# WangYuTum/odometry

Measured on AMD Instinct MI355X. Metric: tracked frames/sec (1241x376, 4-level pyramid), higher is better.
Workload: dtype f32

## Files before the change

### include/odometry_hip.h

```cpp
#ifndef ODOMETRY_HIP_H
#define ODOMETRY_HIP_H

#include <stddef.h>
#include <stdint.h>

#ifdef __cplusplus
extern "C" {
#endif

typedef struct odo_ctx odo_ctx;
typedef struct odo_pyr odo_pyr;
typedef struct odo_lm odo_lm;
typedef struct odo_depth odo_depth;
typedef struct odo_tracker odo_tracker;
typedef struct odo_camera odo_camera;
typedef struct odo_map odo_map;
typedef struct odo_volume odo_volume;
typedef struct odo_rgbd_frontend odo_rgbd_frontend;

typedef struct {
  float f0, cx0, cy0;
} odo_intrinsics;

enum { ODO_PYR_IMAGE = 0, ODO_PYR_DEPTH = 1 };
// ... 69 lines not shown
int odo_lm_time_eval(odo_lm* lm, const odo_pyr* kf_img, const odo_pyr* kf_dep, const odo_pyr* cur_img, int level,
                     const float T_colmajor[16], int reps, float* mean_us, float* min_us, double* algorithmic_bytes,
                     int* n_points);
int odo_lm_time_eval_batch(int n, odo_lm* const* lms, const odo_pyr* const* kf_img, const odo_pyr* const* kf_dep,
                           const odo_pyr* const* cur_img, int level, const float T_colmajor[16], int reps, float* mean_us,
                           float* min_us, double* algorithmic_bytes, int* n_points_total);
int odo_lm_event_timing(odo_lm* lm, int on);
int odo_lm_event_stats(odo_lm* lm, double* total_us, long* launches, long* active_launches,
                       double* algorithmic_bytes);
int odo_lm_event_stats2(odo_lm* lm, double* coarse_us, long* coarse_launches);
int odo_lm_event_stats_ex(odo_lm* lm, double out[12]);
enum { ODO_SAMPLE_FLOOR = 0, ODO_SAMPLE_BILINEAR = 1 };
int odo_lm_set_sampling(odo_lm* lm, int sampling);
int odo_lm_set_mode(odo_lm* lm, int mode);
int odo_lm_points(const odo_lm* lm, int npts[ODO_MAX_LEVELS], int use_list[ODO_MAX_LEVELS]);
int odo_lm_launch_stats(const odo_lm* lm, int* n_active_launches, int* n_total_launches, double* algorithmic_bytes);
int odo_lm_persistent_stats(const odo_lm* lm, int* workgroups, int* fallbacks);
int odo_lm_persistent_backoff(const odo_lm* lm, int* strikes, int* retry_after, int* solves_until_retry);
int odo_lm_tdist_stats(odo_lm* lm, long* multi_launches, int* fallbacks);

int odo_debug_update_stamps(odo_lm* lm, const odo_pyr* kf_img, const odo_pyr* kf_dep, const odo_pyr* cur_img, int level,
                            const float T_colmajor[16], unsigned long long stamps[8]);
int odo_debug_solve(odo_ctx* ctx, const double acc[ODO_NACC], float lambda, float delta[6]);

int odo_depth_create(odo_ctx* ctx, float grad_th, float ssd_th, float photo_th, float min_depth, float max_depth,
                     float lambda, float huber_delta, float precision, int max_iters, int boundary,
                     const odo_intrinsics* K, float baseline, int max_residuals, int max_disparity, int any_size,
                     odo_depth** out);
int odo_depth_compute(odo_depth* d, const float* left, const float* right, int rows, int cols, uint8_t* val,
                      float* disp, float* dep);
// ... 208 lines not shown
```

### odometry_amd/_lib.py

```python
import ctypes as C
import os

_HERE = os.path.dirname(os.path.abspath(__file__))
LIB_PATH = os.environ.get("ODOMETRY_HIP_LIB") or os.path.join(_HERE, "lib", "libodometry_hip.so")

MAX_LEVELS = 8
NACC = 29
PYR_IMAGE, PYR_DEPTH = 0, 1


class Intrinsics(C.Structure):
    _fields_ = [("f0", C.c_float), ("cx0", C.c_float), ("cy0", C.c_float)]


class LmTraceRow(C.Structure):
    _fields_ = [("level", C.c_int), ("iter", C.c_int), ("n_res", C.c_int), ("accepted", C.c_int), ("stop", C.c_int),
                ("err", C.c_float), ("lambda_after", C.c_float), ("delta", C.c_float * 6)]


class TrackerParams(C.Structure):
    _fields_ = [("rows", C.c_int), ("cols", C.c_int), ("levels", C.c_int),
                ("lm_lambda", C.c_float), ("lm_precision", C.c_float), ("lm_max_iters", C.c_int * MAX_LEVELS),
                ("lm_robust", C.c_int), ("lm_huber_delta", C.c_float),
                ("grad_th", C.c_float), ("ssd_th", C.c_float), ("photo_th", C.c_float),
# ... 81 lines not shown
    "odo_lm_trace": (C.c_int, [_vp, C.POINTER(LmTraceRow), C.c_int, _ip]),
    "odo_lm_set_record": (C.c_int, [_vp, C.c_int]),
    "odo_lm_time_eval": (C.c_int, [_vp, _vp, _vp, _vp, C.c_int, _fp, C.c_int, _fp, _fp, _dp, _ip]),
    "odo_lm_time_eval_batch": (C.c_int, [C.c_int, C.POINTER(_vp), C.POINTER(_vp), C.POINTER(_vp), C.POINTER(_vp), C.c_int, _fp, C.c_int, _fp, _fp, _dp, _ip]),
    "odo_lm_event_timing": (C.c_int, [_vp, C.c_int]),
    "odo_lm_event_stats": (C.c_int, [_vp, _dp, C.POINTER(C.c_long), C.POINTER(C.c_long), _dp]),
    "odo_lm_event_stats2": (C.c_int, [_vp, _dp, C.POINTER(C.c_long)]),
    "odo_lm_event_stats_ex": (C.c_int, [_vp, _dp]),
    "odo_lm_solve_begin": (C.c_int, [_vp, _vp, _vp, _vp]),
    "odo_lm_set_idle_callback": (C.c_int, [_vp, _vp, _vp]),
    "odo_lm_candidate_begin": (C.c_int, [_vp, _vp, _vp, _vp, C.c_ulong]),
    "odo_lm_solve_batch": (C.c_int, [C.c_int, C.POINTER(_vp), C.POINTER(_vp), C.POINTER(_vp), C.POINTER(_vp), _fp, C.POINTER(C.c_int)]),
    "odo_lm_set_sampling": (C.c_int, [_vp, C.c_int]),
    "odo_lm_set_mode": (C.c_int, [_vp, C.c_int]),
    "odo_lm_points": (C.c_int, [_vp, _ip, _ip]),
    "odo_lm_launch_stats": (C.c_int, [_vp, _ip, _ip, _dp]),
    "odo_lm_persistent_stats": (C.c_int, [_vp, _ip, _ip]),
    "odo_lm_persistent_backoff": (C.c_int, [_vp, _ip, _ip, _ip]),
    "odo_lm_tdist_stats": (C.c_int, [_vp, C.POINTER(C.c_long), _ip]),
    "odo_debug_update_stamps": (C.c_int, [_vp, _vp, _vp, _vp, C.c_int, _fp, C.POINTER(C.c_ulonglong)]),
    "odo_debug_solve": (C.c_int, [_vp, _dp, C.c_float, _fp]),
    "odo_depth_create": (C.c_int, [_vp] + [C.c_float] * 8 + [C.c_int, C.c_int, C.POINTER(Intrinsics), C.c_float,
                                                          C.c_int, C.c_int, C.c_int, C.POINTER(_vp)]),
    "odo_depth_compute": (C.c_int, [_vp, _fp, _fp, C.c_int, C.c_int, _u8p, _fp, _fp]),
    "odo_depth_compute_dev": (C.c_int, [_vp, _vp, _vp, C.c_int, C.c_int, _vp, _vp, _vp]),
    "odo_depth_prepare_left_dev": (C.c_int, [_vp, _vp, _vp, C.c_int, C.c_int, C.c_ulonglong]),
    "odo_depth_prepare_left_dev_marked": (C.c_int, [_vp, _vp, _vp, C.c_int, C.c_int, C.c_ulonglong, C.c_ulong]),
    "odo_depth_compute_dev_stamped": (C.c_int, [_vp, _vp, _vp, C.c_int, C.c_int, _vp, _vp, _vp, C.c_ulonglong]),
    "odo_depth_compute_begin_dev": (C.c_int, [_vp, _vp, _vp, _vp, C.c_int, C.c_int, _vp, _vp, _vp, C.c_ulonglong, C.c_ulonglong, C.c_ulong]),
    "odo_depth_compute_end_dev": (C.c_int, [_vp, _vp, _vp, C.c_int, C.c_int, _vp, _vp, _vp, C.c_ulonglong, C.c_ulonglong]),
# ... 134 lines not shown
```

### odometry_amd/api.py

```python
import ctypes as C

import numpy as np

from . import _lib as L

_default_ctx = None


class Context:

    def __init__(self, device=0):
        lib = L.load()
        h = C.c_void_p()
        L.check(lib.odo_ctx_create(device, C.byref(h)), "odo_ctx_create")
        self.h = h
        self.lib = lib

    def synchronize(self):
        L.check(self.lib.odo_ctx_synchronize(self.h), "odo_ctx_synchronize")

    def timer_start(self):
        L.check(self.lib.odo_ctx_timer_start(self.h), "timer_start")

    def timer_stop(self):
# ... 193 lines not shown
        L.check(self.ctx.lib.odo_lm_time_eval(self.h, kImagePyr1.h, kDepthPyr1.h, kImagePyr2.h, level, _fp(Tc), reps,
                                              C.byref(mean), C.byref(mn), C.byref(b), C.byref(n)), "odo_lm_time_eval")
        return dict(mean_us=mean.value, min_us=mn.value, bytes=b.value, n_points=n.value)

    def set_sampling(self, bilinear):
        L.check(self.ctx.lib.odo_lm_set_sampling(self.h, 1 if bilinear else 0), "odo_lm_set_sampling")

    def set_mode(self, mode):
        L.check(self.ctx.lib.odo_lm_set_mode(self.h, mode), "odo_lm_set_mode")

    def points(self):
        n = (C.c_int * L.MAX_LEVELS)()
        u = (C.c_int * L.MAX_LEVELS)()
        L.check(self.ctx.lib.odo_lm_points(self.h, n, u), "odo_lm_points")
        return list(n)[:self.n_levels], list(u)[:self.n_levels]

    def launch_stats(self):
        a, t, b = C.c_int(0), C.c_int(0), C.c_double(0)
        L.check(self.ctx.lib.odo_lm_launch_stats(self.h, C.byref(a), C.byref(t), C.byref(b)), "odo_lm_launch_stats")
        return a.value, t.value, b.value

    def persistent_stats(self):
        k, f = C.c_int(0), C.c_int(0)
        L.check(self.ctx.lib.odo_lm_persistent_stats(self.h, C.byref(k), C.byref(f)), "odo_lm_persistent_stats")
        return k.value, f.value

    def tdist_stats(self):
        a, b = C.c_long(0), C.c_int(0)
        L.check(self.ctx.lib.odo_lm_tdist_stats(self.h, C.byref(a), C.byref(b)), "odo_lm_tdist_stats")
        return a.value, b.value
# ... 1055 lines not shown
```

### odometry_amd/csrc/kernels.hip.h

```cpp
#pragma once
#include <hip/hip_runtime.h>
#include "odo_math.h"

#ifndef ODO_PHASE_STAMPS
#define ODO_PHASE_STAMPS 0
#endif
#if ODO_PHASE_STAMPS
#define ODO_DBG(a) ((a).dbg)
#else
#define ODO_DBG(a) ((unsigned long long*)nullptr)
#endif

#ifndef ODO_KERNEL
#define ODO_KERNEL __global__
#define ODO_KERNEL_T __global__
#endif
#ifdef ODO_LM_CHAIN_TU
#define ODO_DEVICE_VAR static __device__
#else
#define ODO_DEVICE_VAR __device__
#endif

namespace odo {

// ... 493 lines not shown
  const int px = (ui - 1 >= 0) ? ui - 1 : 0, nx = (ui + 1 < cols) ? ui + 1 : cols - 1;
  const int py = (vi - 1 >= 0) ? vi - 1 : 0, ny = (vi + 1 < rows) ? vi + 1 : rows - 1;
  const unsigned row = (unsigned)vi * (unsigned)cols, ucols = (unsigned)cols;
  const float tc = ldg_f32(I2_uniform, (row + (unsigned)ui) * 4u), tl = ldg_f32(I2_uniform, (row + (unsigned)px) * 4u),
              tr = ldg_f32(I2_uniform, (row + (unsigned)nx) * 4u), tu = ldg_f32(I2_uniform, ((unsigned)py * ucols + (unsigned)ui) * 4u),
              td = ldg_f32(I2_uniform, ((unsigned)ny * ucols + (unsigned)ui) * 4u);
  const float gx = 0.5f * (tr - tl), gy = 0.5f * (td - tu);
  *r = tc - p.i1;
  J[0] = gx * p.fx_z;
  J[1] = gy * p.fx_z;
  J[2] = gx * p.jw02 + gy * p.jw12;
  J[3] = gx * p.jw03 + gy * p.jw13;
  J[4] = gx * p.jw04 + gy * p.jw14;
  J[5] = gx * p.jw05 + gy * p.jw15;
  return true;
}

ODO_KERNEL void __launch_bounds__(kLmBlock) lm_residual_list_kernel(PointList pl, int n, const float* __restrict__ I2, int rows,
                                                                     int cols, LevelK k, const LmState* __restrict__ st,
                                                                     int expect_level, int robust, float huber_delta,
                                                                     const float* __restrict__ scale_sqr_ptr,
                                                                     double* __restrict__ partials) {
  if (!(st->active != 0 && st->level == expect_level)) return;
  float T[16];
#pragma unroll
  for (int i = 0; i < 16; i++) T[i] = st->T[i];
  const float scale_sqr = (robust == 2) ? *scale_sqr_ptr : 1.0f;
  double acc[ODO_NACC];
#pragma unroll
  for (int q = 0; q < ODO_NACC; q++) acc[q] = 0.0;
// ... 248 lines not shown
template <int T, int S>
__device__ __forceinline__ double rows_accumulate(const float* __restrict__ rows, int rowA, int rowB, int s, double acc) {
  static_assert(S == kRowSub && (T / S) % 4 == 0, "the row layout is built for S sub-lanes");
  constexpr int W = RowBuf<T>::W;
  const float4* A = (const float4*)(rows + rowA * W + s * RowBuf<T>::kStride);
  const float4* B = (const float4*)(rows + rowB * W + s * RowBuf<T>::kStride);
#pragma unroll
  for (int i = 0; i < T / S / 4; i++) {
    const float4 a = A[i], b = B[i];
    acc = fma((double)a.x, (double)b.x, acc);
    acc = fma((double)a.y, (double)b.y, acc);
    acc = fma((double)a.z, (double)b.z, acc);
    acc = fma((double)a.w, (double)b.w, acc);
  }
  return acc;
}

__device__ __forceinline__ double wave_sum64(double v) {
  v += dpp_d<0xB1>(v);
  v += dpp_d<0x4E>(v);
  v += dpp_d<0x141>(v);
  v += dpp_d<0x140>(v);
  const double r0 = readlane_d(v, 0), r1 = readlane_d(v, 16), r2 = readlane_d(v, 32), r3 = readlane_d(v, 48);
  return (r0 + r1) + (r2 + r3);
}
__device__ __forceinline__ float tdist_term(float e2, float sigma_sqr) { return e2 * (1.0f + 200.0f) / (200.0f + e2 / sigma_sqr); }
__device__ __forceinline__ float tdist_next_sigma(double total, int n) { return sqrtf((float)(total / (double)n)); }
__device__ __forceinline__ bool tdist_converged(float nxt, float cur) { return !(fabsf(nxt - cur) >= 1e-3f); }
constexpr int kTdistMaxPasses = 1000;

// ... 625 lines not shown
ODO_KERNEL void __launch_bounds__(kLmBlock) lm_step_kernel(StepArgs a) {
  const StepLaunch q = {a.st_in, a.st_out, a.part_in, a.part_out, a.seq, a.first_of_solve, a.span};
  lm_step_body(a, q);
}
ODO_KERNEL void __launch_bounds__(kLmBlock) lm_step_kernel_batch(const StepArgs* __restrict__ table, int seq, int first_of_solve,
                                                                 unsigned long long* span) {
  const StepArgs& a = table[blockIdx.y];
  const StepLaunch q = {a.st2[seq & 1], a.st2[(seq + 1) & 1], a.part2[seq & 1], a.part2[(seq + 1) & 1], seq, first_of_solve, span};
  lm_step_body(a, q);
}

#ifndef ODO_COARSE_BLOCK
#define ODO_COARSE_BLOCK 512
#endif
constexpr int kCoarseBlock = ODO_COARSE_BLOCK;
constexpr int kCoarseLdsBytes = 2 * RowBuf<kLmBlock>::kBytes;
constexpr int kCoarseMaxPoints = 1024;

constexpr int kCoarseRounds = kCoarseMaxPoints / kCoarseBlock;
constexpr int kCoarseChunks = kCoarseRounds * (kCoarseBlock / kWave);
__device__ __forceinline__ float coarse_tdist_sigma(double (*part)[kCoarseChunks], int* cnt, const float e2[kCoarseRounds],
                                                    const bool valid[kCoarseRounds], int nr) {
  constexpr int kW = kCoarseBlock / kWave;
  const int lane = threadIdx.x & 63, wv = threadIdx.x >> 6;
  int my_cnt[kCoarseRounds];
#pragma unroll
  for (int rd = 0; rd < kCoarseRounds; rd++) my_cnt[rd] = __popcll(__ballot(rd < nr && valid[rd]));
  float sigma = 5.0f;
  int n_total = 0;
  for (int pass = 0; pass < kTdistMaxPasses; pass++) {
#pragma unroll
// ... 76 lines not shown
    __syncthreads();
  }
#if ODO_PHASE_STAMPS
  const unsigned long long w_p1 = (unsigned long long)wall_clock64();
#endif
  lm_fused_prologue(q.st_in, q.part_in, lv_sh, a.n_levels, a.lambda0, a.precision, s_sh, red_sh, acc_sh, (kFull ? a.trace : (LmTraceRow*)nullptr), a.cost_stat, true,
                    kArmed ? arm_pose_sh : (q.first_of_solve ? a.init : nullptr), a.stop_level, (!kArmed && a.chain_in_token) ? a.chain_pose : nullptr);
#if ODO_PHASE_STAMPS
  const unsigned long long w_p2 = (unsigned long long)wall_clock64();
#endif
  LmHot hot;
  lm_hot_load(hot, s_sh);
  if (ODO_DBG(a) && threadIdx.x == 0 && q.seq < 56) ODO_DBG(a)[16 + 2 * q.seq] = wall_clock64();
  unsigned long long c_eval = 0, c_red = 0, c_sm = 0, c_it = 0, c_last = ODO_DBG(a) ? __builtin_readcyclecounter() : 0;
  const unsigned long long c_begin = c_last, w_begin = ODO_DBG(a) ? (unsigned long long)wall_clock64() : 0;
  auto lap = [&](unsigned long long& sum) {
    if (ODO_DBG(a)) { const unsigned long long now = __builtin_readcyclecounter(); sum += now - c_last; c_last = now; }
  };
  static_assert(kCoarseBlock == 2 * kLmBlock, "two 256-point virtual blocks per round");
  constexpr int kS = 8;
  constexpr int kVbMax = (kCoarseMaxPoints + kLmBlock - 1) / kLmBlock;
  __shared__ double part_sh[kVbMax][32];
  __shared__ double sc_part[2][kCoarseChunks];
  __shared__ int sc_cnt[kCoarseChunks];
  const int tl = threadIdx.x & (kLmBlock - 1), half = threadIdx.x >> 8;
  float* rows_sh = (float*)red_sh + half * (kRowFloats * RowBuf<kLmBlock>::W);
  const int my_q = tl / kS, my_s = tl % kS;
  int rowA = 0, rowB = 0;
  if (my_q < ODO_NACC) rows_of_quantity(my_q, &rowA, &rowB);
  PointK cpt[kCoarseRounds];
  bool cpt_ok[kCoarseRounds] = {false, false};
  int cpt_level = -1;
  for (int guard = 0; guard < 4096; guard++) {
    const bool run = (s_sh.active != 0 && s_sh.status == 0 && s_sh.level >= min_level);
    if (!run) break;
    c_it++;
    const StepLevel& L = lv_sh[s_sh.level];
    const float* I2u = lm_uniform_ptr(L.I2);
    float T[16];
#pragma unroll
    for (int i = 0; i < 16; i++) T[i] = s_sh.T[i];
    const int nvb = L.nblk;
    if (s_sh.level != cpt_level) {
      cpt_level = s_sh.level;
#pragma unroll
      for (int rd = 0; rd < kCoarseRounds; rd++) {
        const int vb = 2 * rd + half, idx = vb * kLmBlock + tl;
        cpt_ok[rd] = vb < nvb && idx < L.n;
        if (cpt_ok[rd]) cpt[rd] = load_point(L.pl, idx);
      }
    }
    float td_r[kCoarseRounds] = {0.0f, 0.0f}, td_J[kCoarseRounds][6] = {{0.0f, 0.0f, 0.0f, 0.0f, 0.0f, 0.0f}, {0.0f, 0.0f, 0.0f, 0.0f, 0.0f, 0.0f}};
    bool td_valid[kCoarseRounds] = {false, false};
    float td_scale_sqr = 1.0f;
    if ((kFull && a.robust == 2)) {
      float e2[kCoarseRounds];
#pragma unroll
      for (int rd = 0; rd < kCoarseRounds; rd++) {
        if (cpt_ok[rd]) td_valid[rd] = point_residual_g<kFull>(cpt[rd], T, L.k, I2u, L.rows, L.cols, &td_r[rd], td_J[rd]);
        e2[rd] = td_r[rd] * td_r[rd];
      }
      const float sg = coarse_tdist_sigma(sc_part, sc_cnt, e2, td_valid, (nvb + 1) / 2);
      td_scale_sqr = sg * sg;
    }
#pragma unroll
    for (int vb0 = 0; vb0 < 2 * kCoarseRounds; vb0 += 2) {
      if (vb0 >= nvb) break;
      const int vb = vb0 + half;
      float r = 0.0f, w = 0.0f, J[6] = {0.0f, 0.0f, 0.0f, 0.0f, 0.0f, 0.0f};
      bool valid = false;
      if ((kFull && a.robust == 2)) {
        r = td_r[vb0 / 2]; valid = td_valid[vb0 / 2];
#pragma unroll
        for (int i = 0; i < 6; i++) J[i] = td_J[vb0 / 2][i];
        if (valid) w = robust_weight(r, 2, a.huber_delta, td_scale_sqr);
      } else if (cpt_ok[vb0 / 2]) {
        if (point_residual_g<kFull>(cpt[vb0 / 2], T, L.k, I2u, L.rows, L.cols, &r, J)) {
          w = robust_weight(r, kFull ? a.robust : (a.robust == 1 ? 1 : 0), a.huber_delta, 1.0f);
          valid = true;
        }
      }
      if (vb0 > 0) __syncthreads();
      rows_store_z(rows_sh, RowBuf<kLmBlock>::W, tl, J, w, r, valid);
      __syncthreads();
      if (vb0 == 0) lap(c_eval);
      double accq = 0.0;
      if (vb < nvb) {
        if (my_q < ODO_NACC) accq = rows_accumulate<kLmBlock, kS>(rows_sh, rowA, rowB, my_s, accq);
        accq = rows_butterfly8(accq);
      }
      if (nvb == 1) {
        if (half == 0 && my_q < ODO_NACC && my_s == 0) {
          double v = 0.0;
          v += accq;
          double acc = 0.0;
          acc += v;
#pragma unroll
          for (int g = 1; g < 8; g++) acc += 0.0;
          acc_sh[my_q] = acc;
        }
      } else if (vb < nvb && my_q < ODO_NACC && my_s == 0) {
        part_sh[vb][my_q] = accq;
      }
    }
    __syncthreads();
    if (nvb > 1) {
      const int fq = threadIdx.x & 31, fseg = threadIdx.x >> 5;
      double* fold_sh = red_sh;
      if (fseg < 8) {
        double v = 0.0;
        if (fq < ODO_NACC)
          for (int b = fseg; b < nvb; b += 8) v += part_sh[b][fq];
        fold_sh[fseg * 32 + fq] = v;
      }
      __syncthreads();
      if (threadIdx.x < ODO_NACC) {
        double acc = 0.0;
// ... 12 lines not shown
#endif
  if (threadIdx.x == 0) lm_hot_store(hot, s_sh);
  lm_fused_publish(s_sh, q.st_out, a.host_prog, q.seq, a.token, a.cost_stat, a.out, a.done_flag, a.final_state, chain_out_of(a));
#if ODO_PHASE_STAMPS
  if (ODO_DBG(a) && threadIdx.x == 0) {
    const unsigned long long now = (unsigned long long)wall_clock64();
    g_lm_diag[4] += w_begin - w_entry; g_lm_diag[5] += w_loop_end - w_begin; g_lm_diag[6] += now - w_loop_end;
    g_lm_diag[16] += w_p1 - w_entry; g_lm_diag[17] += w_p2 - w_p1; g_lm_diag[18] += w_begin - w_p2;
    if (g_lm_diag[1] && w_entry > g_lm_diag[1] && w_entry - g_lm_diag[1] < 100000ull) { g_lm_diag[7] += w_entry - g_lm_diag[1]; g_lm_diag[3] += w_entry - g_lm_diag[2]; g_lm_diag[14] += 1; }
    g_lm_diag[0] = now; g_lm_diag[8] += 1;
  }
#endif
  if (ODO_DBG(a) && threadIdx.x == 0) {
    if (q.seq < 56) ODO_DBG(a)[16 + 2 * q.seq + 1] = wall_clock64();
    ODO_DBG(a)[0] += c_eval; ODO_DBG(a)[1] += c_red; ODO_DBG(a)[2] += c_sm; ODO_DBG(a)[3] += c_it;
    ODO_DBG(a)[4] += __builtin_readcyclecounter() - c_begin; ODO_DBG(a)[5] += 1;
    ODO_DBG(a)[6] += (unsigned long long)wall_clock64() - w_begin;
#pragma unroll
    for (int i = 0; i < 4; i++) ODO_DBG(a)[8 + i] += sm_sh[i];
  }
  lm_span_end(q.span);
}

#ifdef ODO_LM_CHAIN_TU
static __global__ void __launch_bounds__(kCoarseBlock) lm_coarse_kernel(StepArgs a, int min_level) {
  const StepLaunch q = {a.st_in, a.st_out, a.part_in, a.part_out, a.seq, a.first_of_solve, a.span};
  lm_coarse_body<false>(a, q, min_level, lm_kernarg_words());
}
static __global__ void __launch_bounds__(kCoarseBlock) lm_coarse_armed_kernel(StepArgs a, int min_level) {
  const StepLaunch q = {a.st_in, a.st_out, a.part_in, a.part_out, a.seq, a.first_of_solve, a.span};
// ... 275 lines not shown
  __syncthreads();
  const bool local = local_sh != 0;
  constexpr int kS = 8;
  const int my_q = tl / kS, my_s = tl % kS;
  int rowA = 0, rowB = 0;
  if (my_q < ODO_NACC) rows_of_quantity(my_q, &rowA, &rowB);
  const int fq = t & 31, fseg = t >> 5;
  PointK pt;
  bool pt_ok = false;
  int pt_level = -1;
  unsigned long long c_eval = 0, c_xchg = 0, c_sm = 0, c_it = 0, c_last = ODO_DBG(a) ? __builtin_readcyclecounter() : 0;
#if ODO_PHASE_STAMPS
  unsigned long long c_first = 0, n_first = 0;
#endif
  const unsigned long long c_begin = c_last, w_begin = ODO_DBG(a) ? (unsigned long long)wall_clock64() : 0;
  auto lap = [&](unsigned long long& sum) {
    if (ODO_DBG(a)) { const unsigned long long now = __builtin_readcyclecounter(); sum += now - c_last; c_last = now; }
  };
  for (int ev = 0; ev < 4096; ev++) {
    const bool run = (s_sh.active != 0 && s_sh.status == 0 && !s_sh.finished && !bail_sh && s_sh.level >= lo_level);
    if (!run) break;
    c_it++;
    const StepLevel& L = lv_sh[s_sh.level];
    const float* I2u = lm_uniform_ptr(L.I2);
    const int nblk = L.nblk;
    const unsigned tag = tag_base + 1u + (unsigned)(ev % 255);
    unsigned long long* buf = xbuf + (size_t)(ev & 1) * kFineRowsMax * kFineGran;
    float T[16];
#pragma unroll
    for (int i = 0; i < 16; i++) T[i] = s_sh.T[i];
#if ODO_PHASE_STAMPS
    const bool first_of_level = (s_sh.level != pt_level);
#endif
    const bool resident = (nblk <= 2 * K) && (L.n <= nblk * kLmBlock);
    if (resident) {
      const int vb = w + half * K;
      if (s_sh.level != pt_level) {
// ... 102 lines not shown
  }
#if ODO_PHASE_STAMPS
  const unsigned long long w_loop_end = (unsigned long long)wall_clock64();
#endif
  if (t == 0) lm_hot_store(hot, s_sh);
  if (bail_sh && t == 0) { s_sh.status = -2; s_sh.active = 0; s_sh.finished = 1; }
  __syncthreads();
  if (publisher) {
    lm_fused_publish(s_sh, q.st_out, a.host_prog, q.seq, a.token, a.cost_stat, a.out, a.done_flag, a.final_state, chain_out_of(a));
#if ODO_PHASE_STAMPS
    const unsigned long long w_published = (unsigned long long)wall_clock64();
#endif
    if (ODO_DBG(a) && t == 0) { ODO_DBG(a)[128] += c_eval; ODO_DBG(a)[129] += c_xchg; ODO_DBG(a)[130] += c_sm; ODO_DBG(a)[131] += c_it; ODO_DBG(a)[132] += 1; ODO_DBG(a)[133] += local ? 1 : 0;
      ODO_DBG(a)[134] += __builtin_readcyclecounter() - c_begin; ODO_DBG(a)[135] += (unsigned long long)wall_clock64() - w_begin;
#pragma unroll
      for (int i = 0; i < 4; i++) ODO_DBG(a)[136 + i] += sm_sh[i]; }
    if (t == 0 && q.span) atomicMax(q.span + 1, (unsigned long long)wall_clock64());
#if ODO_PHASE_STAMPS
    if (ODO_DBG(a) && t == 0) {
      const unsigned long long now = w_published;
      g_lm_diag[2] = w_loop_end;
      g_lm_diag[19] += c_first; g_lm_diag[20] += n_first;
      g_lm_diag[9] += w_begin - w_entry; g_lm_diag[10] += w_loop_end - w_begin; g_lm_diag[11] += now - w_loop_end;
      if (g_lm_diag[0] && w_entry > g_lm_diag[0] && w_entry - g_lm_diag[0] < 100000ull) { g_lm_diag[12] += w_entry - g_lm_diag[0]; g_lm_diag[15] += 1; }
      g_lm_diag[1] = now; g_lm_diag[13] += 1;
    }
#endif
  }
}
ODO_DEVICE_VAR unsigned g_lm_fine_dispatch[2];
__device__ __forceinline__ bool lm_fine_mid_dispatch() {
// ... 873 lines not shown
```

### odometry_amd/csrc/odometry_hip.hip

```cpp
#include <hip/hip_runtime.h>
#include <hip/hip_ext.h>
#include <stdarg.h>
#include <stdio.h>
#include <stdlib.h>
#include <string.h>
#include <chrono>

#include <atomic>
#include <mutex>
#include <new>
#include <thread>
#include <utility>
#include <vector>

#include "../../include/odometry_hip.h"
#include "kernels.hip.h"

using namespace odo;

static thread_local char g_err[512] = "";
static int fail(const char* fmt, ...) {
  va_list ap;
  va_start(ap, fmt);
  vsnprintf(g_err, sizeof(g_err), fmt, ap);
// ... 731 lines not shown
                             odo_lm** out) {
  if (!ctx || !out || !max_iters || !init_colmajor) return fail("odo_lm_create: NULL arg");
  *out = nullptr;
  if (n_levels < 1 || n_levels > ODO_MAX_LEVELS) return fail("odo_lm_create: n_levels %d out of range", n_levels);
  if (robust < 0 || robust > 2) return fail("odo_lm_create: robust must be 0, 1 or 2");
  odo_lm* m = new (std::nothrow) odo_lm();
  if (!m) return fail("out of memory");
  memset(m, 0, sizeof(*m));
  m->ctx = ctx; m->lambda = lambda; m->precision = precision; m->huber_delta = huber_delta;
  m->n_levels = n_levels; m->robust = robust;
  for (int i = 0; i < n_levels; i++) m->max_iters[i] = max_iters[i];
  m->K = K ? *K : kKitti00;
  memcpy(m->init, init_colmajor, sizeof(m->init));
  HIP_OK(hipSetDevice(ctx->device));
  HIP_OK(lm_chain_setup());
  HIP_OK(hipGetSymbolAddress((void**)&m->dispatch_words, HIP_SYMBOL(g_lm_fine_dispatch)));
  HIP_OK(hipMalloc((void**)&m->d_state, sizeof(LmState) * 3));
  m->ust = m->d_state; m->upo = 0;
  m->fuse_dense_max = getenv("ODO_FUSE_DENSE_MAX") ? atoi(getenv("ODO_FUSE_DENSE_MAX")) : 131072;
  HIP_OK(hipMalloc((void**)&m->d_partials, sizeof(double) * 2 * kLmMaxBlocks * ODO_NACC));
  HIP_OK(hipMalloc((void**)&m->d_init, sizeof(float) * 16));
  HIP_OK(hipMalloc((void**)&m->d_out, sizeof(float) * 48));
  HIP_OK(hipMalloc((void**)&m->d_trace, sizeof(LmTraceRow) * kTraceCap));
  m->d_cost = m->d_out + 26;
  HIP_OK(hipMalloc((void**)&m->d_scale, sizeof(float)));
  HIP_OK(hipMalloc((void**)&m->d_ts_xbuf, sizeof(unsigned long long) * kTsXbufWords));
  HIP_OK(hipMemset(m->d_ts_xbuf, 0, sizeof(unsigned long long) * kTsXbufWords));
  HIP_OK(hipMalloc((void**)&m->d_ts_gave_up, 2 * sizeof(int)));
  HIP_OK(hipMemset(m->d_ts_gave_up, 0, 2 * sizeof(int)));
  m->ts_epoch = 0;
// ... 562 lines not shown
          fprintf(stderr, "[lm timeline] launches/Solve %.1f, publisher-block start->end %.2f us per step launch, end->next start "
                  "%.2f us, first start -> last end %.1f us per Solve\n", (double)(n_gap + n_solve) / n_solve,
                  dur_us / (n_gap ? n_gap : 1), gap_us / (n_gap ? n_gap : 1), span_us / n_solve);
      }
      memset(dbg_buf + 16, 0, sizeof(unsigned long long) * 112);
    }
    if (dbg_buf && dbg_buf[5] > 0 && dbg_buf[5] % 100 == 0)
      fprintf(stderr, "[coarse stamps] per iteration: eval %.0f reduce %.0f state-machine %.0f cycles; iterations/launch %.2f, "
              "cycles/launch %.0f\n", (double)dbg_buf[0] / dbg_buf[3], (double)dbg_buf[1] / dbg_buf[3],
              (double)dbg_buf[2] / dbg_buf[3], (double)dbg_buf[3] / dbg_buf[5], (double)dbg_buf[4] / dbg_buf[5]);
    if (dbg_buf && dbg_buf[132] > 0 && dbg_buf[132] % 100 == 0)
      fprintf(stderr, "[fine stamps] per evaluation: eval + publish %.0f gather + fold %.0f state-machine %.0f cycles; evaluations/launch "
              "%.2f, same-XCD launches %.0f %%\n", (double)dbg_buf[128] / dbg_buf[131], (double)dbg_buf[129] / dbg_buf[131],
              (double)dbg_buf[130] / dbg_buf[131], (double)dbg_buf[131] / dbg_buf[132], 100.0 * (double)dbg_buf[133] / dbg_buf[132]);
#if ODO_PHASE_STAMPS
    if (dbg_buf && dbg_buf[5] > 0 && dbg_buf[5] % 500 == 0) {
      unsigned long long g[24];
      lm_chain_diag_read(g);
      if (g[8] && g[13])
        fprintf(stderr, "[wall clock outside the loops] fine loop end -> next coarse entry %.2f us; coarse: previous fine exit -> entry %.2f us, prologue %.2f, loop %.2f, epilogue %.2f; fine: coarse exit -> "
                "entry %.2f us, prologue %.2f, loop %.2f, epilogue %.2f\n", 0.01 * g[3] / (g[14] ? g[14] : 1), 0.01 * g[7] / (g[14] ? g[14] : 1), 0.01 * g[4] / g[8], 0.01 * g[5] / g[8], 0.01 * g[6] / g[8],
                0.01 * g[12] / (g[15] ? g[15] : 1), 0.01 * g[9] / g[13], 0.01 * g[10] / g[13], 0.01 * g[11] / g[13]);
      if (g[20]) fprintf(stderr, "[fine launch] eval + publish of a level's FIRST evaluation: %.0f cycles (%.1f per launch)\n", (double)g[19] / g[20], (double)g[20] / g[13]);
      if (g[8]) fprintf(stderr, "[coarse prologue] entry -> level table in LDS %.2f us, lm_fused_prologue %.2f, hot state %.2f\n", 0.01 * g[16] / g[8], 0.01 * g[17] / g[8], 0.01 * g[18] / g[8]);
    }
#endif
    if (dbg_buf && dbg_buf[5] > 0 && dbg_buf[5] % 100 == 0 && dbg_buf[6] > 0 && dbg_buf[135] > 0)
      fprintf(stderr, "[shader clock] inside the coarse launch %.0f MHz, inside the fine launch %.0f MHz (cycle counter / 100 MHz wall clock)\n",
              (double)dbg_buf[4] / (double)dbg_buf[6] * 100.0, (double)dbg_buf[134] / (double)dbg_buf[135] * 100.0);
    if (dbg_buf && dbg_buf[5] > 0 && dbg_buf[5] % 100 == 0 && dbg_buf[11] > 0)
// ... 886 lines not shown
  if (!m) return fail("odo_lm_tdist_stats: NULL lm");
  HIP_OK(hipSetDevice(m->ctx->device));
  HIP_OK(hipStreamSynchronize(m->ctx->stream));
  int w[2] = {0, 0};
  HIP_OK(hipMemcpy(w, m->d_ts_gave_up, sizeof(w), hipMemcpyDeviceToHost));
  if (multi_launches) *multi_launches = m->ts_multi_launches;
  if (fallbacks) *fallbacks = w[1];
  return 0;
}
extern "C" int odo_lm_persistent_backoff(const odo_lm* m, int* strikes, int* retry_after, int* solves_until_retry) {
  if (!m) return fail("odo_lm_persistent_backoff: NULL lm");
  const int ra = fine_retry_after(m->fine_offs);
  if (strikes) *strikes = m->fine_strikes;
  if (retry_after) *retry_after = ra;
  if (solves_until_retry) *solves_until_retry = (m->fine_k_cfg > 0 && m->fine_k == 0 && m->fine_strikes >= 3) ? (ra - m->fine_clean > 0 ? ra - m->fine_clean : 0) : 0;
  return 0;
}
extern "C" int odo_lm_launch_stats(const odo_lm* m, int* n_active, int* n_total, double* bytes) {
  if (!m) return fail("NULL lm");
  if (n_active) *n_active = m->last_evals;
  if (n_total) *n_total = m->last_launches;
  if (bytes) *bytes = m->last_bytes;
  return 0;
}

__global__ void lm_force_state_kernel(LmState* st, const float* T, int level) {
  if (threadIdx.x == 0) {
    LmState s;
    float m[16];
    for (int i = 0; i < 16; i++) m[i] = T[i];
// ... 637 lines not shown
```

Measured before the change: 4070.

## Evaluate both coarse rounds at once and reduce them together via doubled LDS rows

The coarse LM kernel now computes residuals for both 256-point rounds in one pass, with the two points' projection and gathers interleaved. It stores the rows into two separate LDS buffers and accumulates both with a paired reduction. This removes one barrier and one serial store/reduce round per iteration and adds memory-level parallelism for the image gathers. It doubles the coarse LDS footprint, which could cut occupancy, and also adds per-level phase-stamp instrumentation and a plan query API.

```diff
diff --git a/include/odometry_hip.h b/include/odometry_hip.h
--- a/include/odometry_hip.h
+++ b/include/odometry_hip.h
@@ -107,6 +107,7 @@
 int odo_lm_set_sampling(odo_lm* lm, int sampling);
 int odo_lm_set_mode(odo_lm* lm, int mode);
 int odo_lm_points(const odo_lm* lm, int npts[ODO_MAX_LEVELS], int use_list[ODO_MAX_LEVELS]);
+int odo_lm_plan(const odo_lm* lm, int* coarse_from, int* persistent_from);
 int odo_lm_launch_stats(const odo_lm* lm, int* n_active_launches, int* n_total_launches, double* algorithmic_bytes);
 int odo_lm_persistent_stats(const odo_lm* lm, int* workgroups, int* fallbacks);
 int odo_lm_persistent_backoff(const odo_lm* lm, int* strikes, int* retry_after, int* solves_until_retry);
diff --git a/odometry_amd/_lib.py b/odometry_amd/_lib.py
--- a/odometry_amd/_lib.py
+++ b/odometry_amd/_lib.py
@@ -119,6 +119,7 @@
     "odo_lm_set_sampling": (C.c_int, [_vp, C.c_int]),
     "odo_lm_set_mode": (C.c_int, [_vp, C.c_int]),
     "odo_lm_points": (C.c_int, [_vp, _ip, _ip]),
+    "odo_lm_plan": (C.c_int, [_vp, _ip, _ip]),
     "odo_lm_launch_stats": (C.c_int, [_vp, _ip, _ip, _dp]),
     "odo_lm_persistent_stats": (C.c_int, [_vp, _ip, _ip]),
     "odo_lm_persistent_backoff": (C.c_int, [_vp, _ip, _ip, _ip]),
diff --git a/odometry_amd/api.py b/odometry_amd/api.py
--- a/odometry_amd/api.py
+++ b/odometry_amd/api.py
@@ -231,6 +231,11 @@
         u = (C.c_int * L.MAX_LEVELS)()
         L.check(self.ctx.lib.odo_lm_points(self.h, n, u), "odo_lm_points")
         return list(n)[:self.n_levels], list(u)[:self.n_levels]
+
+    def plan(self):
+        a, b = C.c_int(0), C.c_int(0)
+        L.check(self.ctx.lib.odo_lm_plan(self.h, C.byref(a), C.byref(b)), "odo_lm_plan")
+        return a.value, b.value
 
     def launch_stats(self):
         a, t, b = C.c_int(0), C.c_int(0), C.c_double(0)
diff --git a/odometry_amd/csrc/kernels.hip.h b/odometry_amd/csrc/kernels.hip.h
--- a/odometry_amd/csrc/kernels.hip.h
+++ b/odometry_amd/csrc/kernels.hip.h
@@ -531,6 +531,63 @@
   J[4] = gx * p.jw04 + gy * p.jw14;
   J[5] = gx * p.jw05 + gy * p.jw15;
   return true;
+}
+
+template <bool kMayBilinear>
+__device__ __forceinline__ void point_residual_pair_g(const PointK p[2], const bool ok[2], const float* T, const LevelK& k,
+                                                      const float* I2_uniform, int rows, int cols, int robust, float huber_delta,
+                                                      float r[2], float w[2], float J[2][6], bool valid[2]) {
+  if (kMayBilinear && k.bilinear) {
+#pragma unroll
+    for (int i = 0; i < 2; i++) {
+      r[i] = 0.0f; w[i] = 0.0f; valid[i] = false;
+#pragma unroll
+      for (int a = 0; a < 6; a++) J[i][a] = 0.0f;
+      if (ok[i] && point_residual<true>(p[i], T, k, I2_uniform, rows, cols, &r[i], J[i])) {
+        w[i] = robust_weight(r[i], robust, huber_delta, 1.0f);
+        valid[i] = true;
+      }
+    }
+    return;
+  }
+  unsigned o_c[2], o_l[2], o_r[2], o_u[2], o_d[2];
+#pragma unroll
+  for (int i = 0; i < 2; i++) {
+    const float t0 = ((T[0] * p[i].X + T[4] * p[i].Y) + T[8] * p[i].Z) + T[12];
+    const float t1 = ((T[1] * p[i].X + T[5] * p[i].Y) + T[9] * p[i].Z) + T[13];
+    const float t2 = ((T[2] * p[i].X + T[6] * p[i].Y) + T[10] * p[i].Z) + T[14];
+    const double t2d = (double)t2, y = rcp_refined_d(t2d);
+    const float u = (float)(div_shared_d(k.fl * (double)t0, t2d, y) + (double)k.cx);
+    const float v = (float)(div_shared_d(k.fl * (double)t1, t2d, y) + (double)k.cy);
+    const float fu = floorf(u), fv = floorf(v);
+    valid[i] = ok[i] && (t2 > 0.0f) && (fu < (float)cols) && (fv < (float)rows) && (fu >= 0.0f) && (fv >= 0.0f);
+    const int ui = valid[i] ? (int)fu : 0, vi = valid[i] ? (int)fv : 0;
+    const int px = (ui - 1 >= 0) ? ui - 1 : 0, nx = (ui + 1 < cols) ? ui + 1 : cols - 1;
+    const int py = (vi - 1 >= 0) ? vi - 1 : 0, ny = (vi + 1 < rows) ? vi + 1 : rows - 1;
+    const unsigned row = (unsigned)vi * (unsigned)cols, ucols = (unsigned)cols;
+    o_c[i] = (row + (unsigned)ui) * 4u; o_l[i] = (row + (unsigned)px) * 4u; o_r[i] = (row + (unsigned)nx) * 4u;
+    o_u[i] = ((unsigned)py * ucols + (unsigned)ui) * 4u; o_d[i] = ((unsigned)ny * ucols + (unsigned)ui) * 4u;
+  }
+  float tc[2], tl[2], tr[2], tu[2], td[2];
+#pragma unroll
+  for (int i = 0; i < 2; i++) {
+    tc[i] = ldg_f32(I2_uniform, o_c[i]); tl[i] = ldg_f32(I2_uniform, o_l[i]); tr[i] = ldg_f32(I2_uniform, o_r[i]);
+    tu[i] = ldg_f32(I2_uniform, o_u[i]); td[i] = ldg_f32(I2_uniform, o_d[i]);
+  }
+#pragma unroll
+  for (int i = 0; i < 2; i++) {
+    const float gx = 0.5f * (tr[i] - tl[i]), gy = 0.5f * (td[i] - tu[i]);
+    const float ri = tc[i] - p[i].i1;
+    const float wi = robust_weight(ri, robust, huber_delta, 1.0f);
+    r[i] = valid[i] ? ri : 0.0f;
+    w[i] = valid[i] ? wi : 0.0f;
+    J[i][0] = valid[i] ? gx * p[i].fx_z : 0.0f;
+    J[i][1] = valid[i] ? gy * p[i].fx_z : 0.0f;
+    J[i][2] = valid[i] ? gx * p[i].jw02 + gy * p[i].jw12 : 0.0f;
+    J[i][3] = valid[i] ? gx * p[i].jw03 + gy * p[i].jw13 : 0.0f;
+    J[i][4] = valid[i] ? gx * p[i].jw04 + gy * p[i].jw14 : 0.0f;
+    J[i][5] = valid[i] ? gx * p[i].jw05 + gy * p[i].jw15 : 0.0f;
+  }
 }
 
 ODO_KERNEL void __launch_bounds__(kLmBlock) lm_residual_list_kernel(PointList pl, int n, const float* __restrict__ I2, int rows,
@@ -809,6 +866,31 @@
     acc = fma((double)a.w, (double)b.w, acc);
   }
   return acc;
+}
+template <int T, int S>
+__device__ __forceinline__ void rows_accumulate2(const float* __restrict__ rows0, const float* __restrict__ rows1, int rowA, int rowB, int s,
+                                                 double* acc0, double* acc1) {
+  static_assert(S == kRowSub && (T / S) % 4 == 0, "the row layout is built for S sub-lanes");
+  constexpr int W = RowBuf<T>::W;
+  const int oA = rowA * W + s * RowBuf<T>::kStride, oB = rowB * W + s * RowBuf<T>::kStride;
+  const float4* A0 = (const float4*)(rows0 + oA);
+  const float4* B0 = (const float4*)(rows0 + oB);
+  const float4* A1 = (const float4*)(rows1 + oA);
+  const float4* B1 = (const float4*)(rows1 + oB);
+  double x = *acc0, y = *acc1;
+#pragma unroll
+  for (int i = 0; i < T / S / 4; i++) {
+    const float4 a0 = A0[i], b0 = B0[i], a1 = A1[i], b1 = B1[i];
+    x = fma((double)a0.x, (double)b0.x, x);
+    y = fma((double)a1.x, (double)b1.x, y);
+    x = fma((double)a0.y, (double)b0.y, x);
+    y = fma((double)a1.y, (double)b1.y, y);
+    x = fma((double)a0.z, (double)b0.z, x);
+    y = fma((double)a1.z, (double)b1.z, y);
+    x = fma((double)a0.w, (double)b0.w, x);
+    y = fma((double)a1.w, (double)b1.w, y);
+  }
+  *acc0 = x; *acc1 = y;
 }
 
 __device__ __forceinline__ double wave_sum64(double v) {
@@ -1464,7 +1546,7 @@
 #define ODO_COARSE_BLOCK 512
 #endif
 constexpr int kCoarseBlock = ODO_COARSE_BLOCK;
-constexpr int kCoarseLdsBytes = 2 * RowBuf<kLmBlock>::kBytes;
+constexpr int kCoarseLdsBytes = 4 * RowBuf<kLmBlock>::kBytes;
 constexpr int kCoarseMaxPoints = 1024;
 
 constexpr int kCoarseRounds = kCoarseMaxPoints / kCoarseBlock;
@@ -1571,8 +1653,21 @@
   if (ODO_DBG(a) && threadIdx.x == 0 && q.seq < 56) ODO_DBG(a)[16 + 2 * q.seq] = wall_clock64();
   unsigned long long c_eval = 0, c_red = 0, c_sm = 0, c_it = 0, c_last = ODO_DBG(a) ? __builtin_readcyclecounter() : 0;
   const unsigned long long c_begin = c_last, w_begin = ODO_DBG(a) ? (unsigned long long)wall_clock64() : 0;
+#if ODO_PHASE_STAMPS
+  __shared__ unsigned long long lvl_sh[8][4];
+  int lap_level = 0, lap_slot = 0;
+  if (threadIdx.x == 0)
+    for (int i = 0; i < 32; i++) (&lvl_sh[0][0])[i] = 0;
+#endif
   auto lap = [&](unsigned long long& sum) {
-    if (ODO_DBG(a)) { const unsigned long long now = __builtin_readcyclecounter(); sum += now - c_last; c_last = now; }
+    if (ODO_DBG(a)) {
+      const unsigned long long now = __builtin_readcyclecounter();
+      sum += now - c_last;
+#if ODO_PHASE_STAMPS
+      if (threadIdx.x == 0) { lvl_sh[lap_level & 7][lap_slot] += now - c_last; lap_slot = (lap_slot + 1) % 3; }
+#endif
+      c_last = now;
+    }
   };
   static_assert(kCoarseBlock == 2 * kLmBlock, "two 256-point virtual blocks per round");
   constexpr int kS = 8;
@@ -1582,16 +1677,21 @@
   __shared__ int sc_cnt[kCoarseChunks];
   const int tl = threadIdx.x & (kLmBlock - 1), half = threadIdx.x >> 8;
   float* rows_sh = (float*)red_sh + half * (kRowFloats * RowBuf<kLmBlock>::W);
+  float* rows1_sh = rows_sh + 2 * (kRowFloats * RowBuf<kLmBlock>::W);
   const int my_q = tl / kS, my_s = tl % kS;
   int rowA = 0, rowB = 0;
   if (my_q < ODO_NACC) rows_of_quantity(my_q, &rowA, &rowB);
-  PointK cpt[kCoarseRounds];
+  PointK cpt[kCoarseRounds] = {};
   bool cpt_ok[kCoarseRounds] = {false, false};
   int cpt_level = -1;
   for (int guard = 0; guard < 4096; guard++) {
     const bool run = (s_sh.active != 0 && s_sh.status == 0 && s_sh.level >= min_level);
     if (!run) break;
     c_it++;
+#if ODO_PHASE_STAMPS
+    lap_level = s_sh.level; lap_slot = 0;
+    if (ODO_DBG(a) && threadIdx.x == 0) lvl_sh[lap_level & 7][3] += 1;
+#endif
     const StepLevel& L = lv_sh[s_sh.level];
     const float* I2u = lm_uniform_ptr(L.I2);
     float T[16];
@@ -1607,42 +1707,59 @@
         if (cpt_ok[rd]) cpt[rd] = load_point(L.pl, idx);
       }
     }
-    float td_r[kCoarseRounds] = {0.0f, 0.0f}, td_J[kCoarseRounds][6] = {{0.0f, 0.0f, 0.0f, 0.0f, 0.0f, 0.0f}, {0.0f, 0.0f, 0.0f, 0.0f, 0.0f, 0.0f}};
-    bool td_valid[kCoarseRounds] = {false, false};
-    float td_scale_sqr = 1.0f;
-    if ((kFull && a.robust == 2)) {
-      float e2[kCoarseRounds];
-#pragma unroll
-      for (int rd = 0; rd < kCoarseRounds; rd++) {
-        if (cpt_ok[rd]) td_valid[rd] = point_residual_g<kFull>(cpt[rd], T, L.k, I2u, L.rows, L.cols, &td_r[rd], td_J[rd]);
-        e2[rd] = td_r[rd] * td_r[rd];
-      }
-      const float sg = coarse_tdist_sigma(sc_part, sc_cnt, e2, td_valid, (nvb + 1) / 2);
-      td_scale_sqr = sg * sg;
-    }
-#pragma unroll
-    for (int vb0 = 0; vb0 < 2 * kCoarseRounds; vb0 += 2) {
-      if (vb0 >= nvb) break;
-      const int vb = vb0 + half;
+    if (nvb > 2) {
+      const bool has1 = (2 + half) < nvb;
+      float r[kCoarseRounds] = {0.0f, 0.0f}, w[kCoarseRounds] = {0.0f, 0.0f};
+      float J[kCoarseRounds][6] = {{0.0f, 0.0f, 0.0f, 0.0f, 0.0f, 0.0f}, {0.0f, 0.0f, 0.0f, 0.0f, 0.0f, 0.0f}};
+      bool valid[kCoarseRounds] = {false, false};
+      if ((kFull && a.robust == 2)) {
+        float e2[kCoarseRounds];
+#pragma unroll
+        for (int rd = 0; rd < kCoarseRounds; rd++) {
+          if (cpt_ok[rd]) valid[rd] = point_residual_g<kFull>(cpt[rd], T, L.k, I2u, L.rows, L.cols, &r[rd], J[rd]);
+          e2[rd] = r[rd] * r[rd];
+        }
+        const float sg = coarse_tdist_sigma(sc_part, sc_cnt, e2, valid, (nvb + 1) / 2);
+#pragma unroll
+        for (int rd = 0; rd < kCoarseRounds; rd++)
+          if (valid[rd]) w[rd] = robust_weight(r[rd], 2, a.huber_delta, sg * sg);
+      } else {
+        point_residual_pair_g<kFull>(cpt, cpt_ok, T, L.k, I2u, L.rows, L.cols, kFull ? a.robust : (a.robust == 1 ? 1 : 0), a.huber_delta, r, w, J, valid);
+      }
+      rows_store_z(rows_sh, RowBuf<kLmBlock>::W, tl, J[0], w[0], r[0], valid[0]);
+      if (has1) rows_store_z(rows1_sh, RowBuf<kLmBlock>::W, tl, J[1], w[1], r[1], valid[1]);
+      __syncthreads();
+      lap(c_eval);
+      double accq = 0.0, accq1 = 0.0;
+      if (has1) {
+        if (my_q < ODO_NACC) rows_accumulate2<kLmBlock, kS>(rows_sh, rows1_sh, rowA, rowB, my_s, &accq, &accq1);
+        accq = rows_butterfly8(accq);
+        accq1 = rows_butterfly8(accq1);
+      } else {
+        if (my_q < ODO_NACC) accq = rows_accumulate<kLmBlock, kS>(rows_sh, rowA, rowB, my_s, accq);
+        accq = rows_butterfly8(accq);
+      }
+      if (my_q < ODO_NACC && my_s == 0) {
+        part_sh[half][my_q] = accq;
+        if (has1) part_sh[2 + half][my_q] = accq1;
+      }
+    } else {
       float r = 0.0f, w = 0.0f, J[6] = {0.0f, 0.0f, 0.0f, 0.0f, 0.0f, 0.0f};
       bool valid = false;
+      if (cpt_ok[0] && point_residual_g<kFull>(cpt[0], T, L.k, I2u, L.rows, L.cols, &r, J)) valid = true;
       if ((kFull && a.robust == 2)) {
-        r = td_r[vb0 / 2]; valid = td_valid[vb0 / 2];
-#pragma unroll
-        for (int i = 0; i < 6; i++) J[i] = td_J[vb0 / 2][i];
-        if (valid) w = robust_weight(r, 2, a.huber_delta, td_scale_sqr);
-      } else if (cpt_ok[vb0 / 2]) {
-        if (point_residual_g<kFull>(cpt[vb0 / 2], T, L.k, I2u, L.rows, L.cols, &r, J)) {
-          w = robust_weight(r, kFull ? a.robust : (a.robust == 1 ? 1 : 0), a.huber_delta, 1.0f);
-          valid = true;
-        }
-      }
-      if (vb0 > 0) __syncthreads();
+        const float e2[kCoarseRounds] = {r * r, 0.0f};
+        const bool td_valid[kCoarseRounds] = {valid, false};
+        const float sg = coarse_tdist_sigma(sc_part, sc_cnt, e2, td_valid, 1);
+        if (valid) w = robust_weight(r, 2, a.huber_delta, sg * sg);
+      } else if (valid) {
+        w = robust_weight(r, kFull ? a.robust : (a.robust == 1 ? 1 : 0), a.huber_delta, 1.0f);
+      }
       rows_store_z(rows_sh, RowBuf<kLmBlock>::W, tl, J, w, r, valid);
       __syncthreads();
-      if (vb0 == 0) lap(c_eval);
+      lap(c_eval);
       double accq = 0.0;
-      if (vb < nvb) {
+      if (half < nvb) {
         if (my_q < ODO_NACC) accq = rows_accumulate<kLmBlock, kS>(rows_sh, rowA, rowB, my_s, accq);
         accq = rows_butterfly8(accq);
       }
@@ -1656,8 +1773,8 @@
           for (int g = 1; g < 8; g++) acc += 0.0;
           acc_sh[my_q] = acc;
         }
-      } else if (vb < nvb && my_q < ODO_NACC && my_s == 0) {
-        part_sh[vb][my_q] = accq;
+      } else if (my_q < ODO_NACC && my_s == 0) {
+        part_sh[half][my_q] = accq;
       }
     }
     __syncthreads();
@@ -1700,6 +1817,9 @@
   if (ODO_DBG(a) && threadIdx.x == 0) {
     if (q.seq < 56) ODO_DBG(a)[16 + 2 * q.seq + 1] = wall_clock64();
     ODO_DBG(a)[0] += c_eval; ODO_DBG(a)[1] += c_red; ODO_DBG(a)[2] += c_sm; ODO_DBG(a)[3] += c_it;
+#if ODO_PHASE_STAMPS
+    for (int i = 0; i < 32; i++) ODO_DBG(a)[144 + i] += (&lvl_sh[0][0])[i];
+#endif
     ODO_DBG(a)[4] += __builtin_readcyclecounter() - c_begin; ODO_DBG(a)[5] += 1;
     ODO_DBG(a)[6] += (unsigned long long)wall_clock64() - w_begin;
 #pragma unroll
@@ -2005,13 +2125,30 @@
   unsigned long long c_first = 0, n_first = 0;
 #endif
   const unsigned long long c_begin = c_last, w_begin = ODO_DBG(a) ? (unsigned long long)wall_clock64() : 0;
+#if ODO_PHASE_STAMPS
+  __shared__ unsigned long long lvl_sh[8][4];
+  int lap_level = 0, lap_slot = 0;
+  if (t == 0)
+    for (int i = 0; i < 32; i++) (&lvl_sh[0][0])[i] = 0;
+#endif
   auto lap = [&](unsigned long long& sum) {
-    if (ODO_DBG(a)) { const unsigned long long now = __builtin_readcyclecounter(); sum += now - c_last; c_last = now; }
+    if (ODO_DBG(a)) {
+      const unsigned long long now = __builtin_readcyclecounter();
+      sum += now - c_last;
+#if ODO_PHASE_STAMPS
+      if (t == 0) { lvl_sh[lap_level & 7][lap_slot] += now - c_last; lap_slot = (lap_slot + 1) % 3; }
+#endif
+      c_last = now;
+    }
   };
   for (int ev = 0; ev < 4096; ev++) {
     const bool run = (s_sh.active != 0 && s_sh.status == 0 && !s_sh.finished && !bail_sh && s_sh.level >= lo_level);
     if (!run) break;
     c_it++;
+#if ODO_PHASE_STAMPS
+    lap_level = s_sh.level; lap_slot = 0;
+    if (ODO_DBG(a) && t == 0) lvl_sh[lap_level & 7][3] += 1;
+#endif
     const StepLevel& L = lv_sh[s_sh.level];
     const float* I2u = lm_uniform_ptr(L.I2);
     const int nblk = L.nblk;
@@ -2144,7 +2281,11 @@
     if (ODO_DBG(a) && t == 0) { ODO_DBG(a)[128] += c_eval; ODO_DBG(a)[129] += c_xchg; ODO_DBG(a)[130] += c_sm; ODO_DBG(a)[131] += c_it; ODO_DBG(a)[132] += 1; ODO_DBG(a)[133] += local ? 1 : 0;
       ODO_DBG(a)[134] += __builtin_readcyclecounter() - c_begin; ODO_DBG(a)[135] += (unsigned long long)wall_clock64() - w_begin;
 #pragma unroll
-      for (int i = 0; i < 4; i++) ODO_DBG(a)[136 + i] += sm_sh[i]; }
+      for (int i = 0; i < 4; i++) ODO_DBG(a)[136 + i] += sm_sh[i];
+#if ODO_PHASE_STAMPS
+      for (int i = 0; i < 32; i++) ODO_DBG(a)[176 + i] += (&lvl_sh[0][0])[i];
+#endif
+    }
     if (t == 0 && q.span) atomicMax(q.span + 1, (unsigned long long)wall_clock64());
 #if ODO_PHASE_STAMPS
     if (ODO_DBG(a) && t == 0) {
diff --git a/odometry_amd/csrc/odometry_hip.hip b/odometry_amd/csrc/odometry_hip.hip
--- a/odometry_amd/csrc/odometry_hip.hip
+++ b/odometry_amd/csrc/odometry_hip.hip
@@ -769,6 +769,8 @@
   memcpy(m->init, init_colmajor, sizeof(m->init));
   HIP_OK(hipSetDevice(ctx->device));
   HIP_OK(lm_chain_setup());
+  HIP_OK(hipFuncSetAttribute((const void*)lm_coarse_kernel_batch, hipFuncAttributeMaxDynamicSharedMemorySize, kCoarseLdsBytes));
+  HIP_OK(hipFuncSetAttribute((const void*)lm_coarse_full_kernel_batch, hipFuncAttributeMaxDynamicSharedMemorySize, kCoarseLdsBytes));
   HIP_OK(hipGetSymbolAddress((void**)&m->dispatch_words, HIP_SYMBOL(g_lm_fine_dispatch)));
   HIP_OK(hipMalloc((void**)&m->d_state, sizeof(LmState) * 3));
   m->ust = m->d_state; m->upo = 0;
@@ -1361,6 +1363,15 @@
               "%.2f, same-XCD launches %.0f %%\n", (double)dbg_buf[128] / dbg_buf[131], (double)dbg_buf[129] / dbg_buf[131],
               (double)dbg_buf[130] / dbg_buf[131], (double)dbg_buf[131] / dbg_buf[132], 100.0 * (double)dbg_buf[133] / dbg_buf[132]);
 #if ODO_PHASE_STAMPS
+    if (dbg_buf && dbg_buf[5] > 0 && dbg_buf[5] % 100 == 0)
+      for (int l = 0; l < 8; l++) {
+        const unsigned long long* c = dbg_buf + 144 + 4 * l;
+        const unsigned long long* f = dbg_buf + 176 + 4 * l;
+        if (c[3]) fprintf(stderr, "[coarse stamps] level %d: eval %.0f reduce %.0f state-machine %.0f cycles per iteration; iterations/launch %.2f\n", l,
+                          (double)c[0] / c[3], (double)c[1] / c[3], (double)c[2] / c[3], (double)c[3] / dbg_buf[5]);
+        if (f[3] && dbg_buf[132]) fprintf(stderr, "[fine stamps] level %d: eval + publish %.0f gather + fold %.0f state-machine %.0f cycles per evaluation; "
+                          "evaluations/launch %.2f\n", l, (double)f[0] / f[3], (double)f[1] / f[3], (double)f[2] / f[3], (double)f[3] / dbg_buf[132]);
+      }
     if (dbg_buf && dbg_buf[5] > 0 && dbg_buf[5] % 500 == 0) {
       unsigned long long g[24];
       lm_chain_diag_read(g);
@@ -2277,6 +2288,12 @@
   if (strikes) *strikes = m->fine_strikes;
   if (retry_after) *retry_after = ra;
   if (solves_until_retry) *solves_until_retry = (m->fine_k_cfg > 0 && m->fine_k == 0 && m->fine_strikes >= 3) ? (ra - m->fine_clean > 0 ? ra - m->fine_clean : 0) : 0;
+  return 0;
+}
+extern "C" int odo_lm_plan(const odo_lm* m, int* coarse_from, int* persistent_from) {
+  if (!m) return fail("odo_lm_plan: NULL lm");
+  if (coarse_from) *coarse_from = m->job.min_level;
+  if (persistent_from) *persistent_from = m->job.fine_lo;
   return 0;
 }
 extern "C" int odo_lm_launch_stats(const odo_lm* m, int* n_active, int* n_total, double* bytes) {
```

After: 4105 (median of 6 runs). Within noise of the previous version (+0.8%).
